# HelixDB/helix-db

Hardware: AMD Instinct MI355X
Metric: QPS @ recall@10>=0.95, 1Mx768 fp32; achieved HBM GB/s vs roofline (higher is better)
Workload: dtype f32; 1 GPU; configs[1]: 1000000x768 f32 per GPU, HNSW M=16/M0=32 ef_search=128 k=10, batch=1024 queries, squared-L2, strict-exhaustive beam (bit-exact vs reference CPU path), steps issued round-robin on 4 execution lanes; dataset=embedding, rows_per_gpu=1000000, rows_total=1000000, dim=768, batch=1024, k=10, ef_search=128, lanes=4, distinct_query_batches=25, exchange=single GPU, parallelism=1 GPU

## Files before the change

helix-db_amd/csrc/hvx_api.hip:

```cpp
#include <hip/hip_runtime.h>

#include <algorithm>
#include <atomic>
#include <cmath>
#include <cstdarg>
#include <cstdio>
#include <cstdlib>
#include <cstring>
#include <mutex>
#include <string>
#include <thread>
#include <vector>

#include "hvx_host.h"
#include "hvx_flat_mfma.h"

using namespace hvx;

namespace {
thread_local std::string g_err;
}

namespace hvx {
int fail(int code, const char *fmt, ...) {
// ... 88 lines not shown
    HIP_TRY(hipSetDevice(ix->device));
    HIP_TRY(hipStreamSynchronize(ix->stream));
    return HVX_OK;
}

extern "C" int hvx_index_set_occupancy(hvx_index *ix, uint32_t queries_per_simd) {
    if (!ix) return fail(HVX_ERR_INVARIANT, "null index");
    if (queries_per_simd != 1 && queries_per_simd != 2) return fail(HVX_ERR_K_RANGE, "occupancy must be 1 or 2 queries per SIMD");
    std::lock_guard<std::mutex> lock(ix->mu);
    ix->occupancy = queries_per_simd;
    return HVX_OK;
}

extern "C" int hvx_runtime_prepare(uint32_t hw_queues) {
    if (hw_queues == 0) hw_queues = 2;
    if (hw_queues > 2) return fail(HVX_ERR_K_RANGE, "hardware queue count %u outside 1..2", hw_queues);
    char buf[16];
    snprintf(buf, sizeof(buf), "%u", hw_queues);
    if (setenv("GPU_MAX_HW_QUEUES", buf, 0) != 0) return fail(HVX_ERR_INVARIANT, "setenv(GPU_MAX_HW_QUEUES) failed");
    return HVX_OK;
}

extern "C" int hvx_index_set_option(hvx_index *ix, uint32_t option, uint32_t value) {
    if (!ix) return fail(HVX_ERR_INVARIANT, "null index");
    if (option >= HVX_OPT_COUNT) return fail(HVX_ERR_INVARIANT, "unknown option %u", option);
    if (option == HVX_OPT_WAVE_LOG2CAP && value != 0 && (value < 7 || value > 15)) return fail(HVX_ERR_K_RANGE, "visited-table size must be 2^7 .. 2^15 slots");
    if (option == HVX_OPT_FLAT_FIRST_CHUNK && value != 0 && value < 1024) return fail(HVX_ERR_K_RANGE, "the first chunk holds at least 1024 rows");
    if (option == HVX_OPT_HNSW_PAIR && value > 3) return fail(HVX_ERR_K_RANGE, "pair kernel selector is 0 (one query per SIMD handles), 1 (never), 2 (always) or 3 (always, one gatherer)");
    if (option == HVX_OPT_FLAT_TILE_BUILD && value > 4) return fail(HVX_ERR_K_RANGE, "tile build is 0 (default: two 256-thread workgroups per CU; fp8 rows on the MX-scaled fp8 matrix instruction), 1, 2 or 3 (as 0) or 4 (as 0 with fp8 codes widened to bf16)");
    if (option == HVX_OPT_HNSW_SHADOW_PRUNE && value > 1) return fail(HVX_ERR_K_RANGE, "shadow pruning selector is 0 (on where a shadow exists) or 1 (off)");
    if (option == HVX_OPT_FLAT_NO_SMALLB && value > 2) return fail(HVX_ERR_K_RANGE, "small-batch selector is 0 (streaming kernels), 1 (never) or 2 (register-fragment build only)");
    if (option == HVX_OPT_FLAT_TILE_BUILD && value != 4) value = 0;
    if (option == HVX_OPT_DELETE_SEQUENTIAL && value != 1) value = 0;
    std::lock_guard<std::mutex> lock(ix->mu);
    ix->opt[option] = value;
    return HVX_OK;
}

extern "C" int hvx_index_read_rows_device(const hvx_index *cix, uint64_t row0, uint64_t n, float *d_out) {
    if (!cix || (!d_out && n)) return fail(HVX_ERR_INVARIANT, "null argument");
    hvx_index *ix = const_cast<hvx_index *>(cix);
    if (row0 > ix->dev.n || n > ix->dev.n - row0) return fail(HVX_ERR_INVARIANT, "rows [%llu, %llu) outside the index (%u rows)", (unsigned long long)row0,
                                                               (unsigned long long)(row0 + n), ix->dev.n);
    std::lock_guard<std::mutex> lock(ix->mu);
    HIP_TRY(hipSetDevice(ix->device));
    HIP_TRY(launch_read_rows(ix->dev, row0, n, d_out, ix->stream));
    HIP_TRY(hipStreamSynchronize(ix->stream));
    return HVX_OK;
}

extern "C" uint32_t hvx_index_last_scan_path(const hvx_index *ix) { return ix ? ix->last_scan_path : 0u; }

extern "C" void *hvx_index_stream(const hvx_index *ix) { return ix ? (void *)ix->stream : nullptr; }

// ... 557 lines not shown
    a.k = k;
    a.ef = ef;
    a.out_ids = d_ids;
    a.out_scores = d_scores;
    a.out_counts = d_counts;
    a.out_status = d_status;
    a.qstats = d_qstats ? d_qstats : ix->d_qstats;
    a.tie_flags = ix->d_tie;
    a.rerun_list = ix->d_tie + ix->max_batch;
    a.rerun_ctl = ix->d_tie + 2 * (size_t)ix->max_batch;
    a.prof = nullptr;
    a.wave_clock = nullptr;
    a.adaptive = ad ? 1u : 0u;
    a.ad = ad ? *ad : AdaptArgs{};
    a.build_nodes = nullptr;
    a.build_ef_upper = 0;
    a.only_flagged = 0;
    a.occupancy = ix->occupancy;
    a.pair = ix->opt[HVX_OPT_HNSW_PAIR] >= 2u || (ix->opt[HVX_OPT_HNSW_PAIR] == 0u && ix->occupancy != 2u) ? 1u : 0u;
    a.pair_gatherers = ix->opt[HVX_OPT_HNSW_PAIR] == 3u ? 1u : 0u;
    a.log2cap = ix->opt[HVX_OPT_WAVE_LOG2CAP];
    a.shadow = nullptr;
    a.shadow_err = nullptr;
    if (ad) {
        if (!hnsw_wave_adaptive_supported(a))
            return fail(HVX_ERR_UNSUPPORTED, "the non-strict search arms serve f32 rows of any dimension / metric (bf16 rows: dim in "
                        "{128,256,512,768,1024,1536}, cosine / Euclidean), neighbour rows <= 64 ids, ef <= 800");
        if (ix->bitmap_dirty) {
            HIP_TRY(hipMemsetAsync(ix->d_bitmap, 0, (size_t)ix->max_batch * ix->words_per_query * 4, ix->stream));
            ix->bitmap_dirty = false;
        }
        const bool ad_prof = tuning_env("HVX_WAVE_PROF") != nullptr && hnsw_wave_supported(a) && ix->occupancy != 2u;
        if (ad_prof) {
            if (!ix->d_prof && ix->dalloc((void **)&ix->d_prof, (size_t)ix->max_batch * 80)) return HVX_ERR_DEVICE;
            a.prof = ix->d_prof;
        }
        hipEvent_t e0 = nullptr, e1 = nullptr;
        pick_events(ix, timed, &e0, &e1, &a.wave_clock);
        if (e0) HIP_TRY(hipEventRecord(e0, ix->stream));
        HIP_TRY(launch_hnsw_wave(a, b, ix->stream));
        if (e1) HIP_TRY(hipEventRecord(e1, ix->stream));
        if (ad_prof) {
            std::vector<unsigned long long> h((size_t)b * 10);
            HIP_TRY(hipMemcpyAsync(h.data(), ix->d_prof, h.size() * 8, hipMemcpyDeviceToHost, ix->stream));
            HIP_TRY(hipStreamSynchronize(ix->stream));
            double acc[10] = {0, 0, 0, 0, 0, 0, 0, 0, 0, 0};
            for (uint32_t i = 0; i < b; ++i)
                for (int j = 0; j < 10; ++j) acc[j] += (double)h[(size_t)i * 10 + j];
            fprintf(stderr, "[hvx prof, non-strict] per query: row-wait %.0f  visited-claim %.0f  decide+select %.0f  gather+fma %.0f  predict %.0f  admit %.0f  (layer-0 loop %.0f) cycles\n",
                    acc[0] / b, acc[1] / b, acc[6] / b, acc[2] / b, acc[3] / b, acc[4] / b, acc[7] / b);
        }
        return HVX_OK;
    }
    const bool prof = tuning_env("HVX_WAVE_PROF") != nullptr;
    if (prof) {
        if (!ix->d_prof && ix->dalloc((void **)&ix->d_prof, (size_t)ix->max_batch * 80)) return HVX_ERR_DEVICE;
        a.prof = ix->d_prof;
    }
    const bool force_general = ix->opt[HVX_OPT_HNSW_GENERAL_KERNEL] != 0;
    const bool wave = !(force_general && ix->dev.dtype == HVX_F32) && hnsw_wave_supported(a);
    if (!wave && ix->dev.dtype != HVX_F32)
        return fail(HVX_ERR_UNSUPPORTED, ix->dev.dtype == HVX_FP8_E4M3 ? "fp8 rows serve the exact scan only (HNSW over fp8 rows is not built)"
                    : "bf16 rows are served by the one-wavefront-per-query kernel only (dim in {128,256,512,768,1024,1536}, rows <= 64 ids, ef <= 800)");
    if (ix->bitmap_dirty) {
        HIP_TRY(hipMemsetAsync(ix->d_bitmap, 0, (size_t)ix->max_batch * ix->words_per_query * 4, ix->stream));
        ix->bitmap_dirty = false;
    }
    if (wave && (ix->occupancy == 2 || prof) && ix->dev.dtype == HVX_F32 && ix->dev.metric == kL2 && !ix->opt[HVX_OPT_HNSW_SHADOW_PRUNE]) {
        uint16_t *sh = nullptr;
        float *se = nullptr;
        int rc = shadow_catch_up(ix, &sh, &se);
        if (rc) return rc;
        a.shadow = sh;
        a.shadow_err = se;
    }
    hipEvent_t e0 = nullptr, e1 = nullptr;
    pick_events(ix, timed, &e0, &e1, &a.wave_clock);
    if (e0) HIP_TRY(hipEventRecord(e0, ix->stream));
    if (wave) {
        HIP_TRY(launch_hnsw_wave(a, b, ix->stream));
        if (prof) {
            std::vector<unsigned long long> h((size_t)b * 10);
            HIP_TRY(hipMemcpyAsync(h.data(), ix->d_prof, h.size() * 8, hipMemcpyDeviceToHost, ix->stream));
            HIP_TRY(hipStreamSynchronize(ix->stream));
            double acc[10] = {0, 0, 0, 0, 0, 0, 0, 0, 0, 0};
            for (uint32_t i = 0; i < b; ++i)
                for (int j = 0; j < 10; ++j) acc[j] += (double)h[(size_t)i * 10 + j];
            fprintf(stderr, "[hvx prof] per query: row-wait %.0f  visited+shadow %.0f  gather+fma %.0f  predict %.0f  admit %.0f  (layer-0 loop %.0f) cycles;"
                            " fresh-candidate predictions %.1f  row-prefetch hits %.1f;  full-beam rows: shadow-pruned %.1f  scored in f32 %.1f"
                            " (pruned share %.4f)\n",
                    acc[0] / b, acc[1] / b, acc[2] / b, acc[3] / b, acc[4] / b, acc[7] / b, acc[5] / b, acc[6] / b, acc[8] / b, acc[9] / b,
                    acc[8] + acc[9] > 0 ? acc[8] / (acc[8] + acc[9]) : 0.0);
        }
    } else {
        HIP_TRY(launch_hnsw_search(a, b, ix->stream));
        ix->bitmap_dirty = true;
    }
    if (e1) HIP_TRY(hipEventRecord(e1, ix->stream));
    return HVX_OK;
}

extern "C" int hvx_index_timing_begin(hvx_index *ix, uint32_t capacity) {
    if (!ix) return fail(HVX_ERR_INVARIANT, "null index");
    std::lock_guard<std::mutex> lock(ix->mu);
    HIP_TRY(hipSetDevice(ix->device));
    while (ix->ring.size() < (size_t)capacity * 2) {
        hipEvent_t e;
        HIP_TRY(hipEventCreate(&e));
        ix->ring.push_back(e);
    }
    if (capacity > ix->wclk_cap) {
        int rc = ix->regrow((void **)&ix->d_wclk, (size_t)capacity * ix->max_batch * 2 * sizeof(unsigned long long));
        if (rc) return rc;
        ix->wclk_cap = capacity;
    }
// ... 322 lines not shown
```

helix-db_amd/csrc/hvx_hnsw_wave.h:

```cpp
#pragma once
#include <type_traits>

#include "hvx_beam.h"
#include "hvx_device.h"
#include "hvx_kernels.h"
#include "hvx_shadow_bound.h"

namespace hvx {

constexpr uint32_t kTabEmpty = 0xFFFFFFFFu;
constexpr uint32_t kTentativeBit = 0x80000000u;
constexpr uint32_t kHashedBit = 0x40000000u;

__device__ __forceinline__ uint32_t umin_dpp_row(uint32_t v) {
    uint32_t t;
    t = (uint32_t)__builtin_amdgcn_mov_dpp((int)v, 0xB1, 0xF, 0xF, true); v = v < t ? v : t;
    t = (uint32_t)__builtin_amdgcn_mov_dpp((int)v, 0x4E, 0xF, 0xF, true); v = v < t ? v : t;
    t = (uint32_t)__builtin_amdgcn_mov_dpp((int)v, 0x141, 0xF, 0xF, true); v = v < t ? v : t;
    t = (uint32_t)__builtin_amdgcn_mov_dpp((int)v, 0x140, 0xF, 0xF, true); v = v < t ? v : t;
    return v;
}
__device__ __forceinline__ uint32_t wave_umin(uint32_t v) {
    v = umin_dpp_row(v);
    uint32_t a = __builtin_amdgcn_readlane(v, 0), b = __builtin_amdgcn_readlane(v, 16);
// ... 375 lines not shown
        else if (!topk_ready) d.threshold = 1u;
        else d.threshold = (uint32_t)__builtin_popcountll(__ballot(delta <= brk_lane));
    }
    return d;
}

__device__ __forceinline__ float candidate_probability_fn(uint32_t kind, float base, uint32_t sim_bits, bool has_thr, uint32_t thr) {
    if (kind != 2u) return base;
    if (base <= 0.0f || base >= 1.0f) return base;
    const float sr = (float)(sim_bits < 64u ? sim_bits : 64u) / 64.0f;
    const float tr = has_thr ? (float)thr / 64.0f : 0.0f;
    const float t = __builtin_fmaxf(sr - tr, 0.0f);
    const float u = (1.0f - base) * t;
    return rs_clampf(base + u, base, 1.0f);
}

template <uint32_t METRIC, int R, int NK, bool BF, bool PROF, bool AD, bool ST, int OCC, bool BUILD>
__device__ __forceinline__ void hnsw_wave_query(const HnswArgs &a, const uint32_t vcap, const uint32_t q) {
    constexpr bool GEN = NK == 0;
    constexpr int NL = GEN ? 1 : (BF ? NK / 2 : NK);
    constexpr int P = NL <= 8 ? 2 : 1;
    constexpr bool kCosBfBig = BF && METRIC == kCosine && NL >= 24;
    constexpr bool kWide4 = OCC == 1 && 4 * P * NL <= 96 && !kCosBfBig;
    constexpr bool kWide2 = OCC == 1 || (2 * P * NL <= 48 && !kCosBfBig && !(AD && ((METRIC == kCosine && 2 * P * NL > 32) || (BF && 2 * P * NL >= 32))));
    extern __shared__ __attribute__((aligned(16))) char smem[];
    const DevIndex &ix = a.ix;
    const int lane = (int)threadIdx.x, grp = lane >> 3, j = lane & 7;
    const int slot = chunk_slot(j);

    Visited V;
    V.tab = reinterpret_cast<uint32_t *>(smem);
    V.cap = vcap;
    V.limit = OCC == 1 ? V.cap - (V.cap >> 2) : V.cap - (V.cap >> 3);
    V.words = a.words_per_query;
    V.bm = a.bitmap + (size_t)q * a.words_per_query;
    V.bm2 = (AD && a.bitmap2) ? a.bitmap2 + (size_t)q * a.words_per_query : nullptr;
    V.count = 0;
    V.spilled = false;
    uint32_t *fr_id = V.tab + V.cap;
    float *fr_d = reinterpret_cast<float *>(fr_id + 64);
    float *qs = fr_d + 64;
    uint32_t *rng_buf = reinterpret_cast<uint32_t *>(qs + (GEN ? ix.ld : (uint32_t)NK * 32u));

    const unsigned long long wclk0 = (a.wave_clock && !a.only_flagged) ? wall_clock64() : 0ull;
    const uint32_t status_in = BUILD ? 0u : (a.qstatus ? a.qstatus[q] : 0u);
    if (status_in != 0u || !ix.has_entry) {
        if (lane == 0) {
// ... 59 lines not shown
            else if (kWide4 && rem > 16u * P) { pass(std::integral_constant<int, kWide4 ? 3 * P : P>{}, f0, nf); f0 += 24u * P; }
            else if (kWide2 && rem > 8u * P) { pass(std::integral_constant<int, kWide2 ? 2 * P : P>{}, f0, nf); f0 += 16u * P; }
            else { pass(std::integral_constant<int, P>{}, f0, nf); f0 += 8u * P; }
        }
        __syncthreads();
    };
    auto score_one = [&](uint32_t node) __attribute__((always_inline)) -> float {
        if constexpr (GEN) {
            return __uint_as_float(__builtin_amdgcn_readlane(__float_as_uint(generic_distance(node)), 0));
        } else {
            uint32_t nd[1] = {node};
            float o[1];
            Gather<NK, 1, BF> g;
            gather_issue<NK, 1, BF, 1, METRIC == kCosine>(ix, nd, slot, g);
            gather_consume<METRIC, NK, 1, BF>(ix, qs, g, nd, slot, qhdr, qglobal, o);
            return __uint_as_float(__builtin_amdgcn_readlane(__float_as_uint(o[0]), 0));
        }
    };
    constexpr bool SP = !AD && !BUILD && !BF && !GEN && METRIC == kL2 && R <= 6 && (OCC == 2 || PROF);
    constexpr int SL = SP ? NK / 2 : 1;
    constexpr int kFL = (kWide4 ? 4 * P : (kWide2 ? 2 * P : P)) * NL;
    constexpr int kSWmax = !SP ? 1 : 8 * SL * 4 <= kFL * 3 ? 8 : 4 * SL * 4 <= kFL * 3 ? 4 : 3 * SL * 4 <= kFL * 3 ? 3 : 2 * SL * 4 <= kFL * 3 ? 2 : 1;
    const bool shadow_on = SP && a.shadow != nullptr;
    auto shadow_pass = [&](auto width, uint32_t f0, uint32_t nf) __attribute__((always_inline)) {
        constexpr int W = decltype(width)::value;
        uint32_t nd[W];
        uint4 x[W][SL];
        float e[W];
#pragma unroll
        for (int p = 0; p < W; ++p) {
            const uint32_t f = f0 + (uint32_t)(p * 8 + grp);
            nd[p] = fr_id[f < nf ? f : f0];
        }
#pragma unroll
        for (int p = 0; p < W; ++p) e[p] = a.shadow_err[nd[p]];
#pragma unroll
        for (int p = 0; p < W; ++p) {
            const uint4 *rp = reinterpret_cast<const uint4 *>(a.shadow + (size_t)nd[p] * ix.dim) + j;
#pragma unroll
            for (int k = 0; k < SL; ++k) x[p][k] = rp[k * 8];
        }
        __builtin_amdgcn_sched_barrier(0);
        float4 acc[W];
#pragma unroll
        for (int p = 0; p < W; ++p) acc[p] = make_float4(0.f, 0.f, 0.f, 0.f);
        const float4 *qp = reinterpret_cast<const float4 *>(qs) + 2 * j;
#pragma unroll
        for (int k = 0; k < SL; ++k) {
            const float4 q0 = qp[16 * k], q1 = qp[16 * k + 1];
#pragma unroll
            for (int p = 0; p < W; ++p) {
                const uint4 w = x[p][k];
                fma_chunk<kL2>(acc[p], q0, make_float4(__uint_as_float(w.x << 16), __uint_as_float(w.x & 0xFFFF0000u),
                                                       __uint_as_float(w.y << 16), __uint_as_float(w.y & 0xFFFF0000u)));
                fma_chunk<kL2>(acc[p], q1, make_float4(__uint_as_float(w.z << 16), __uint_as_float(w.z & 0xFFFF0000u),
                                                       __uint_as_float(w.w << 16), __uint_as_float(w.w & 0xFFFF0000u)));
            }
        }
#pragma unroll
        for (int p = 0; p < W; ++p) {
            float r = (acc[p].x + acc[p].y) + (acc[p].z + acc[p].w);
            r += __shfl_xor(r, 1, 8);
            r += __shfl_xor(r, 2, 8);
            r += __shfl_xor(r, 4, 8);
            const uint32_t f = f0 + (uint32_t)(p * 8 + grp);
            if (f < nf && j == 0) fr_d[f] = shadow_l2_lower_bound(r, e[p], ix.dim);
        }
    };
    auto shadow_prune = [&](uint32_t nf, float thr) __attribute__((always_inline)) -> uint32_t {
        if constexpr (SP) {
            uint32_t f0 = 0;
            while (f0 < nf) {
                const uint32_t rem = nf - f0;
                if (kSWmax >= 8 && rem > 32u) { shadow_pass(std::integral_constant<int, kSWmax >= 8 ? 8 : 1>{}, f0, nf); f0 += 64u; }
                else if (kSWmax >= 4 && rem > 24u) { shadow_pass(std::integral_constant<int, kSWmax >= 4 ? 4 : 1>{}, f0, nf); f0 += 32u; }
                else if (kSWmax >= 3 && rem > 16u) { shadow_pass(std::integral_constant<int, kSWmax >= 3 ? 3 : 1>{}, f0, nf); f0 += 24u; }
                else if (kSWmax >= 2 && rem > 8u) { shadow_pass(std::integral_constant<int, kSWmax >= 2 ? 2 : 1>{}, f0, nf); f0 += 16u; }
                else { shadow_pass(std::integral_constant<int, 1>{}, f0, nf); f0 += 8u; }
            }
            __syncthreads();
            const bool in = (uint32_t)lane < nf;
            const uint32_t id = in ? fr_id[lane] : kSentinel;
            const bool keep = in && !(fr_d[in ? lane : 0] > thr);
            const unsigned long long km = __ballot(keep);
            __syncthreads();
            if (keep) fr_id[__builtin_popcountll(km & ((1ull << lane) - 1ull))] = id;
            __syncthreads();
            return (uint32_t)__builtin_popcountll(km);
        } else {
            return nf;
        }
    };
    auto frontier_from = [&](uint32_t nid, uint32_t &deg) __attribute__((always_inline)) -> uint32_t {
        const bool valid = nid != kSentinel;
        const bool isnew = V.insert(nid, valid, lane);
        const unsigned long long um = __ballot(isnew);
        deg = (uint32_t)__builtin_popcountll(__ballot(valid));
        if (isnew) fr_id[__builtin_popcountll(um & ((1ull << lane) - 1ull))] = nid;
        __syncthreads();
        return (uint32_t)__builtin_popcountll(um);
    };

    uint32_t vslot = 0;
    bool vhashed = false;
    auto frontier_claim = [&](uint32_t nid, uint32_t &deg, unsigned long long &um) __attribute__((always_inline)) -> uint32_t {
        const bool valid = nid != kSentinel;
        const bool unseen = V.claim(nid, valid, lane, vslot, vhashed);
// ... 54 lines not shown
    }

    Beam<R> S;
    uint32_t st_exp = 0, st_nb = 0, st_vl = 0, st_dc = 0;
    bool tie_overflow = false;
    uint32_t bl = beam_top;
    auto load_row = [&](uint32_t c) __attribute__((always_inline)) -> uint32_t {
        if (!BUILD || bl == 0u) return (uint32_t)lane < ix.s0 ? ix.l0[(size_t)c * ix.s0 + (uint32_t)lane] : kSentinel;
        const uint32_t base = ix.up_base[c];
        return (uint32_t)lane < ix.su ? ix.up[(size_t)(base + bl - 1u) * ix.su + (uint32_t)lane] : kSentinel;
    };
    uint32_t dropped_unexpanded = 0;
    uint32_t ef = a.ef;
    uint32_t pf_id = kSentinel, pf_row = kSentinel;
    uint32_t pf_hash_for = kSentinel;
    unsigned long long pf_hash = 0ull;
    const bool want_hash = AD && a.ad.filtering != 0u;
    auto prefetch_hash = [&]() __attribute__((always_inline)) {
        if (AD && want_hash && pf_id != kSentinel && pf_hash_for != pf_id) {
            pf_hash = pf_row != kSentinel ? a.ad.node_hash[pf_row] : 0ull;
            pf_hash_for = pf_id;
        }
    };
    unsigned long long pt[10] = {0, 0, 0, 0, 0, 0, 0, 0, 0, 0}, t0 = 0, t1 = 0, t_begin = 0;
    auto tick = [&](int phase, bool wait) __attribute__((always_inline)) {
        if (PROF) {
            if (wait) asm volatile("s_waitcnt vmcnt(0) lgkmcnt(0)" ::: "memory");
            t1 = __builtin_readcyclecounter();
            pt[phase] += t1 - t0;
            t0 = t1;
        }
    };
    AdaptState A;
    QueryRngT<(OCC == 2 ? kRngWordsOcc2 : kRngWords)> G;
    uint64_t qh = 0;
    float brk_lane = -1.0f;
    if (AD) {
        A.fill = A.win_ex = A.win_filt = A.win_exp = A.bstate = A.bremain = A.reads = 0u;
        A.st = hvx_adaptive_stats{};
        qh = a.ad.qhash[q];
        brk_lane = a.ad.thr_break[lane];
        G.buf = rng_buf;
        const uint64_t ep = ix.ids[cur], efw = (uint64_t)a.ef;
        G.seed(qh ^ ((ep << 17) | (ep >> 47)) ^ ((efw << 7) | (efw >> 57)));
    }
  for (;;) {
    S.init();
// ... 21 lines not shown
            }
            break;
        }
        ++st_exp;
        const float dc = S.score_at(pos);
        const uint32_t c = S.id_at(pos);
        const uint32_t wlen = S.count < ef ? S.count : ef;
        float wmax = S.score_at(wlen - 1);
        if (AD && ST) { A.st.effective_beam_len_sum += wlen + A.fill; A.st.effective_beam_len_samples += 1u; }
        if (wlen + (AD ? A.fill : 0u) >= ef && dc > wmax) break;
        S.mark_expanded(pos, lane);

        uint32_t nid;
        if (c == pf_id) { nid = pf_row; if (PROF && !AD) pt[6] += 1; }
        else nid = load_row(c);
        tick(0, true);
        unsigned long long nh = 0ull;
        if (AD && want_hash) nh = c == pf_hash_for ? pf_hash : (nid != kSentinel ? a.ad.node_hash[nid] : 0ull);
        uint32_t deg;
        unsigned long long um = 0ull;
        uint32_t nf = AD ? frontier_claim(nid, deg, um) : frontier_from(nid, deg);
        st_nb += deg;
        tick(1, true);
        const uint32_t p2 = S.first_unexpanded(lane);
        uint32_t e2 = kSentinel, row2 = kSentinel;
        float s2 = inf;
        if (p2 < S.count) {
            e2 = S.id_at(p2);
            s2 = S.score_at(p2);
            row2 = load_row(e2);
        }
        pf_id = e2;
        pf_row = row2;
        if (nf == 0) { prefetch_hash(); continue; }
        if (AD) {
            const AdaptArgs &P = a.ad;
            const uint32_t nf0 = nf;
            const uint32_t node = nid;
            const unsigned long long node_h = nh;
            const bool unseen = (um >> lane) & 1ull;
            const uint32_t frank = (uint32_t)__builtin_popcountll(um & ((1ull << lane) - 1ull));
            const uint32_t kt = a.k > 1u ? a.k : 1u;
            const float delta = S.score_at((kt < wlen ? kt : wlen) - 1u);
            const AdaptDecision D = adapt_decide(P, A, ef, wlen >= kt, wlen, nf0, dc, delta, brk_lane);
            if (ST) A.st.simhash_bypass_trigger_low_yield += (D.trigger & 2u) ? 1u : 0u;
            if (ST) A.st.simhash_bypass_trigger_budget += (D.trigger & 1u) ? 1u : 0u;
            if (ST) A.st.active_sampling_ratio_sum += (double)D.base_p;
            if (ST) A.st.active_sampling_ratio_samples += 1u;
            if (ST && D.filter) { A.st.active_simhash_threshold_sum += D.threshold; A.st.active_simhash_threshold_samples += 1u; }
            bool keep = unseen;
            const bool pre_enabled = D.pre_kind != 0u;
            if (pre_enabled) {
                if (D.pre_p <= 0.0f) keep = false;
                else if (D.pre_p < 1.0f) {
                    G.ensure(lane);
                    keep = keep && G.below(G.pos + frank, D.pre_p);
                    G.pos += nf0;
// ... 50 lines not shown
                deferred = pass;
            }
            if (D.samp_p > 0.0f && !__ballot(sampled) && __ballot(deferred)) {
                const uint32_t best = 64u - wave_umin(deferred ? 64u - sim : 0xFFFFFFFFu);
                unsigned long long bm = __ballot(deferred & (sim == best));
                uint32_t idx = G.choose_index((uint32_t)__builtin_popcountll(bm), lane);
                while (idx--) bm &= bm - 1ull;
                sampled = (uint32_t)lane == (uint32_t)__builtin_ctzll(bm);
            }
            V.commit(node, sampled | vfail, vslot);
            const bool acc = sampled;
            const unsigned long long am = __ballot(acc);
            if (ST) A.st.simhash_passed_after_sampling += (uint32_t)__builtin_popcountll(__ballot(sampled));
            if (acc) fr_id[__builtin_popcountll(am & ((1ull << lane) - 1ull))] = node;
            __syncthreads();
            nf = (uint32_t)__builtin_popcountll(am);
            tick(6, true);
            if (nf == 0) { prefetch_hash(); continue; }
        }
        st_vl += nf;
        st_dc += nf;
        if (shadow_on && wlen >= ef) {
            const uint32_t nf_all = nf;
            nf = shadow_prune(nf, wmax);
            if (PROF) { pt[8] += nf_all - nf; pt[9] += nf; }
            tick(1, true);
        }
        score_frontier(nf);
        prefetch_hash();
        tick(2, true);
        const float d_l = (uint32_t)lane < nf ? fr_d[lane] : inf;
        const uint32_t id_l = (uint32_t)lane < nf ? fr_id[lane] : kSentinel;
        __syncthreads();
        {
            const uint32_t wl0 = (S.count < ef ? S.count : ef) + (AD ? A.fill : 0u);
            const bool adm = ((uint32_t)lane < nf) & ((d_l < wmax) | (wl0 < ef)) & (d_l >= 0.f) & (d_l < inf);
            const uint32_t key = adm ? __float_as_uint(d_l) : 0xFFFFFFFFu;
            const uint32_t kmin = wave_umin(key);
            if (kmin != 0xFFFFFFFFu && __uint_as_float(kmin) < s2) {
                const uint32_t pred = __builtin_amdgcn_readlane(id_l, (uint32_t)__builtin_ctzll(__ballot(key == kmin)));
                pf_id = pred;
                pf_row = load_row(pred);
                if (PROF) pt[5] += 1;
            }
        }
        tick(3, false);
        {
            float dv = d_l;
            const bool okv = (uint32_t)lane >= nf || score_valid(dv);
            if (__ballot(!okv)) { bad_score = true; break; }
            const uint32_t wl_in = (S.count < ef ? S.count : ef) + (AD ? A.fill : 0u);
            unsigned long long todo = __ballot(((uint32_t)lane < nf) & ((dv < wmax) | (wl_in < ef)));
            while (todo) {
                const uint32_t f = (uint32_t)__builtin_ctzll(todo);
                todo &= todo - 1ull;
                const float d = __uint_as_float(__builtin_amdgcn_readlane(__float_as_uint(dv), f));
                const uint32_t wl = (S.count < ef ? S.count : ef) + (AD ? A.fill : 0u);
                if (d < wmax || wl < ef) {
                    if (AD) A.fill -= (wl >= ef && A.fill > 0u) ? 1u : 0u;
                    float ds = 0.f;
                    const bool drop = S.insert(d, __builtin_amdgcn_readlane(id_l, f), lane, ds);
                    const uint32_t wl2 = S.count < ef ? S.count : ef;
                    wmax = S.score_at(wl2 - 1);
                    if (drop) {
                        ++dropped_unexpanded;
                        if (!(ds > wmax)) tie_overflow = true;
                    }
                }
            }
        }
        prefetch_hash();
        if (PROF) { t1 = __builtin_readcyclecounter(); pt[4] += t1 - t0; t0 = t1; }
    }
    if (!BUILD) break;
    {
        const uint32_t wl = bad_score ? 0u : (S.count < ef ? S.count : ef);
        const uint32_t outn = wl < a.k ? wl : a.k;
        const size_t slot0 = ((size_t)bl * gridDim.x + q) * a.k;
#pragma unroll
        for (int r = 0; r < R; ++r) {
            const uint32_t e = (uint32_t)r * 64u + (uint32_t)lane;
            if (e < outn) {
                a.out_ids[slot0 + e] = (uint64_t)(S.id[r] & ~kExpandedBit);
                a.out_scores[slot0 + e] = S.sc[r];
            }
        }
        if (lane == 0) a.out_counts[(size_t)bl * gridDim.x + q] = outn;
        if (bad_score || bl == 0u) break;
        cur = S.id_at(0) & ~kExpandedBit;
        cur_d = S.score_at(0);
        have_d = true;
        --bl;
    }
  }
    if (PROF && a.prof && lane == 0) {
        pt[7] = __builtin_readcyclecounter() - t_begin;
        for (int i = 0; i < 10; ++i) a.prof[(size_t)q * 10 + i] = pt[i];
    }

    uint32_t outn = 0;
    if (!BUILD && !bad_score) {
        const uint32_t ef = a.ef;
        const uint32_t wl = S.count < ef ? S.count : ef;
        outn = wl < a.k ? wl : a.k;
#pragma unroll
        for (int r = 0; r < R; ++r) {
            const uint32_t e = (uint32_t)r * 64u + (uint32_t)lane;
            if (e < outn) {
                a.out_ids[(size_t)q * a.k + e] = ix.ids[S.id[r] & ~kExpandedBit];
                a.out_scores[(size_t)q * a.k + e] = S.sc[r];
            }
        }
    }
    if (V.spilled) {
        for (uint32_t w = (uint32_t)lane; w < V.words; w += 64) { V.bm[w] = 0u; if (V.bm2) V.bm2[w] = 0u; }
    }
    if (lane == 0) {
        if (a.wave_clock && !a.only_flagged) { a.wave_clock[2 * (size_t)q] = wclk0; a.wave_clock[2 * (size_t)q + 1] = wall_clock64(); }
        if (!BUILD) a.out_counts[q] = outn;
        if (a.out_status) a.out_status[q] = bad_score ? 8u  : 0u;
// ... 112 lines not shown
```

helix-db_amd/csrc/hvx_kernels.h:

```cpp
#pragma once
#include <hip/hip_runtime.h>
#include <stdint.h>

#include "../../include/helix_vec.h"
#include "hvx_device.h"

namespace hvx {

struct AdaptArgs {
    const uint64_t *node_hash;
    const uint64_t *qhash;
    const float *thr_break;
    hvx_adaptive_stats *stats;
    uint32_t filtering;
    uint32_t configured;
    uint32_t sampling;
    float ratio;
    float pre_override;
    uint32_t count_reads;
    uint32_t read_budget;
    uint32_t bypass_windowed;
    uint32_t min_frontier, window_expansions;
    float min_filter_rate;
};

struct HnswArgs {
    DevIndex ix;
    const float *queries;
    const uint32_t *qstatus;
    const float *qhdr;
    uint32_t *bitmap;
    uint32_t *bitmap2;
    uint32_t words_per_query;
    uint32_t k, ef;
    uint64_t *out_ids;
    float *out_scores;
    uint32_t *out_counts;
    uint32_t *out_status;
    hvx_query_stats *qstats;
    uint32_t *tie_flags;
    uint32_t *rerun_list;
    uint32_t *rerun_ctl;
    unsigned long long *prof;
    unsigned long long *wave_clock;
    uint32_t adaptive;
    const uint32_t *build_nodes;
    uint32_t build_ef_upper;
    uint32_t only_flagged;
    uint32_t occupancy;
    uint32_t pair;
    uint32_t pair_gatherers;
    uint32_t log2cap;
    const uint16_t *shadow;
    const float *shadow_err;
    AdaptArgs ad;
};

// ... 55 lines not shown
```

helix-db_amd/pyhvx/__init__.py:

```python
from __future__ import annotations

import ctypes as C
import os
from dataclasses import dataclass

import numpy as np

_HERE = os.path.dirname(os.path.abspath(__file__))
LIB_PATH = os.environ.get("HVX_LIB_PATH") or os.path.join(os.path.dirname(_HERE), "libhelix_vec_gfx950.so")

COSINE, EUCLIDEAN, MANHATTAN = 0, 1, 2
F32, BF16, FP8_E4M3 = 0, 1, 2
KERNEL_SCALAR, KERNEL_SSE, KERNEL_AVX, KERNEL_AVX_FMA, KERNEL_NEON = 0, 1, 2, 3, 4
OK, ERR_DIMENSION, ERR_NONFINITE, ERR_ZERO_NORM, ERR_MAGNITUDE, ERR_K_RANGE, ERR_CANDIDATE_LIMIT, \
    ERR_DEVICE, ERR_INVARIANT, ERR_UNSUPPORTED, PENDING, ERR_BUSY, ERR_TIMEOUT = range(13)
DIR_OUT, DIR_IN, DIR_BOTH = 0, 1, 2

_STATUS_NAMES = {
    1: "InvalidDimension", 2: "InvalidVectorComponent", 3: "ZeroNormCosineVector",
    4: "ComponentMagnitudeExceeded", 5: "Query(result count / beam width out of range)",
    6: "Query(too many restricted candidates)", 7: "Device", 8: "InvariantViolation", 9: "Unsupported",
}


# ... 94 lines not shown
                                          "unsorted_entries", "self_loops", "out_of_range_ids", "holes", "level_violations",
                                          "degree_overflow_rows", "unreachable_l0")] + \
               [(n, C.c_uint32) for n in ("max_degree_l0", "max_degree_up", "bfs_levels_l0", "max_layer", "has_entry", "reserved")]

    def as_dict(self):
        return {n: int(getattr(self, n)) for n, _ in self._fields_ if n != "reserved"}


class AdaptiveStats(C.Structure):
    _fields_ = [(n, C.c_uint32) for n in (
        "simhash_filtered", "simhash_examined", "simhash_passed_before_sampling", "simhash_passed_after_sampling",
        "pre_simhash_sample_kept", "pre_simhash_sample_dropped", "simhash_bypass_expansions",
        "simhash_skipped_candidates", "simhash_bypass_trigger_budget", "simhash_bypass_trigger_low_yield",
        "active_simhash_threshold_sum", "active_simhash_threshold_samples", "effective_beam_len_sum",
        "effective_beam_len_samples", "active_sampling_ratio_samples", "rng_words", "txn_get_simhash_filter")] + \
        [("active_sampling_ratio_sum", C.c_double)]

    def as_dict(self):
        return {k: getattr(self, k) for k, _ in self._fields_}


OPT_HNSW_GENERAL_KERNEL, OPT_WAVE_LOG2CAP, OPT_FLAT_FORCE_VALU, OPT_FLAT_FIRST_CHUNK, OPT_FLAT_NO_TILE, OPT_FLAT_NO_FILTER, \
    OPT_FLAT_NO_FAST, OPT_FLAT_TILE_BUILD, OPT_FLAT_NO_SMALLB, OPT_HNSW_PAIR, OPT_DELETE_SEQUENTIAL, OPT_RESTRICTED_DIRECT, \
    OPT_RESTRICTED_EXACT_MIB, OPT_FLAT_NO_TAIL, OPT_HNSW_SHADOW_PRUNE = range(15)
PATH_VALU, PATH_MFMA_128, PATH_TILE_256, PATH_FILTERED, PATH_FULL_SPLIT, PATH_VALU_FALLBACK_QUERIES, PATH_WIDENED, \
    PATH_PAIR_OVERFLOW_REPEAT, PATH_SMALL_BATCH, PATH_DIRECT, PATH_EXACT_TAIL = 1, 2, 4, 8, 16, 32, 64, 128, 256, 512, 1024
RESTRICTED_AUTO, RESTRICTED_EXACT, RESTRICTED_FILTERED, RESTRICTED_REFERENCE_PLAN = 0, 1, 2, 3
TERM_NONE, TERM_EXHAUSTED, TERM_BEAM_COMPLETE, TERM_ROUTING_BUDGET, TERM_BRIDGE_BUDGET, TERM_VECTOR_BUDGET = range(6)


class RestrictedParams(C.Structure):
    _fields_ = [(n, C.c_uint32) for n in ("k", "ef", "strategy", "beam_percent", "directory_enabled", "explicit_budgets", "ef_filtered",
                                          "routing_rows", "bridge_rows", "vector_payloads", "sampled_seeds", "directory_seeds")]

    @classmethod
    def new(cls, k, ef, *, strategy=RESTRICTED_REFERENCE_PLAN, beam_percent=150, directory=True, **budgets):
        p = cls(k=k, ef=ef, strategy=strategy, beam_percent=beam_percent, directory_enabled=1 if directory else 0)
        if budgets:
            p.explicit_budgets = 1
            p.strategy = RESTRICTED_FILTERED
            for name in ("ef_filtered", "routing_rows", "bridge_rows", "vector_payloads", "sampled_seeds", "directory_seeds"):
                setattr(p, name, int(budgets.pop(name)))
            assert not budgets, budgets
        return p


    @classmethod
# ... 1222 lines not shown
```

include/helix_vec.h:

```cpp
#ifndef HELIX_VEC_H
#define HELIX_VEC_H

#include <stddef.h>
#include <stdint.h>

#ifdef __cplusplus
extern "C" {
#endif

typedef struct hvx_index hvx_index;
typedef struct hvx_csr hvx_csr;

enum hvx_metric { HVX_COSINE_HALF = 0, HVX_L2_SQUARED = 1, HVX_MANHATTAN = 2 };
enum hvx_dtype { HVX_F32 = 0, HVX_BF16 = 1, HVX_FP8_E4M3 = 2 };
enum hvx_float_kernel {
    HVX_KERNEL_SCALAR = 0,
    HVX_KERNEL_SSE = 1,
    HVX_KERNEL_AVX = 2,
    HVX_KERNEL_AVX_FMA = 3,
    HVX_KERNEL_NEON = 4
};

enum hvx_status {
    HVX_OK = 0,
// ... 51 lines not shown
                             hvx_index **out);
void hvx_index_free(hvx_index *);
int hvx_index_sync(const hvx_index *);
void *hvx_index_stream(const hvx_index *);
int hvx_index_read_rows_device(const hvx_index *, uint64_t row0, uint64_t n, float *d_out);
int hvx_index_set_stream(hvx_index *, void *hip_stream);
int hvx_index_fork(const hvx_index *, hvx_index **out);
enum hvx_option {
    HVX_OPT_HNSW_GENERAL_KERNEL = 0,
    HVX_OPT_WAVE_LOG2CAP = 1,
    HVX_OPT_FLAT_FORCE_VALU = 2,
    HVX_OPT_FLAT_FIRST_CHUNK = 3,
    HVX_OPT_FLAT_NO_TILE = 4,
    HVX_OPT_FLAT_NO_FILTER = 5,
    HVX_OPT_FLAT_NO_FAST = 6,
    HVX_OPT_FLAT_TILE_BUILD = 7,
    HVX_OPT_FLAT_NO_SMALLB = 8,
    HVX_OPT_HNSW_PAIR = 9,
    HVX_OPT_DELETE_SEQUENTIAL = 10,
    HVX_OPT_RESTRICTED_DIRECT = 11,
    HVX_OPT_RESTRICTED_EXACT_MIB = 12,
    HVX_OPT_FLAT_NO_TAIL = 13,
    HVX_OPT_HNSW_SHADOW_PRUNE = 14,
    HVX_OPT_COUNT = 15
};
int hvx_index_set_option(hvx_index *, uint32_t option, uint32_t value);
enum hvx_scan_path {
    HVX_PATH_VALU = 1, HVX_PATH_MFMA_128 = 2, HVX_PATH_TILE_256 = 4, HVX_PATH_FILTERED = 8, HVX_PATH_FULL_SPLIT = 16,
    HVX_PATH_VALU_FALLBACK_QUERIES = 32, HVX_PATH_WIDENED = 64,
    HVX_PATH_SMALL_BATCH = 256,
    HVX_PATH_PAIR_OVERFLOW_REPEAT = 128,
    HVX_PATH_DIRECT = 512,
    HVX_PATH_EXACT_TAIL = 1024
};
uint32_t hvx_index_last_scan_path(const hvx_index *);
int hvx_index_set_occupancy(hvx_index *, uint32_t queries_per_simd);
int hvx_index_timing_begin(hvx_index *, uint32_t capacity);
int hvx_index_timing_collect(hvx_index *, float *out_ms, uint32_t cap, uint32_t *out_n);
int hvx_index_wave_clocks(hvx_index *, uint64_t *out, uint32_t cap_launches, uint32_t rows_per_launch, uint32_t *out_n);

int hvx_search_batch(const hvx_index *, const float *queries , uint32_t b, uint32_t k,
                     uint32_t ef, uint64_t *out_ids , float *out_scores ,
                     uint32_t *out_counts , uint32_t *out_status ,
                     hvx_stats *stats );
int hvx_search_batch_device(const hvx_index *, const float *d_queries, uint32_t b, uint32_t k,
                            uint32_t ef, uint64_t *d_out_ids, float *d_out_scores,
                            uint32_t *d_out_counts, uint32_t *d_out_status,
// ... 293 lines not shown
```

Baseline: 1.430 million queries/s.

## Defer small survivor gathers into the next step's shadow pre-pass

When few frontier rows survive shadow pruning and their lower bounds cannot beat the next candidate, the full-precision gather for those survivors is postponed. It is issued alongside the next iteration's shadow-row loads, which removes a separate dependent memory round trip per step. The deferred scores are admitted into the beam before that step's pruning, and the next expansion is re-predicted afterwards. This adds register pressure and control complexity in the hot loop. It also narrows the wide-gather setting for one cosine configuration and adds profiling counters plus an option to turn the deferral off.

```diff
diff --git a/helix-db_amd/csrc/hvx_api.hip b/helix-db_amd/csrc/hvx_api.hip
--- a/helix-db_amd/csrc/hvx_api.hip
+++ b/helix-db_amd/csrc/hvx_api.hip
@@ -134,14 +134,15 @@
 }
 
 extern "C" int hvx_index_set_option(hvx_index *ix, uint32_t option, uint32_t value) {
-    if (!ix) return fail(HVX_ERR_INVARIANT, "null index");
     if (option >= HVX_OPT_COUNT) return fail(HVX_ERR_INVARIANT, "unknown option %u", option);
     if (option == HVX_OPT_WAVE_LOG2CAP && value != 0 && (value < 7 || value > 15)) return fail(HVX_ERR_K_RANGE, "visited-table size must be 2^7 .. 2^15 slots");
     if (option == HVX_OPT_FLAT_FIRST_CHUNK && value != 0 && value < 1024) return fail(HVX_ERR_K_RANGE, "the first chunk holds at least 1024 rows");
     if (option == HVX_OPT_HNSW_PAIR && value > 3) return fail(HVX_ERR_K_RANGE, "pair kernel selector is 0 (one query per SIMD handles), 1 (never), 2 (always) or 3 (always, one gatherer)");
     if (option == HVX_OPT_FLAT_TILE_BUILD && value > 4) return fail(HVX_ERR_K_RANGE, "tile build is 0 (default: two 256-thread workgroups per CU; fp8 rows on the MX-scaled fp8 matrix instruction), 1, 2 or 3 (as 0) or 4 (as 0 with fp8 codes widened to bf16)");
     if (option == HVX_OPT_HNSW_SHADOW_PRUNE && value > 1) return fail(HVX_ERR_K_RANGE, "shadow pruning selector is 0 (on where a shadow exists) or 1 (off)");
+    if (option == HVX_OPT_HNSW_DEFER_SURVIVORS && value > 1) return fail(HVX_ERR_K_RANGE, "deferred survivors selector is 0 (on where the shadow pre-pass is on) or 1 (off)");
     if (option == HVX_OPT_FLAT_NO_SMALLB && value > 2) return fail(HVX_ERR_K_RANGE, "small-batch selector is 0 (streaming kernels), 1 (never) or 2 (register-fragment build only)");
+    if (!ix) return fail(HVX_ERR_INVARIANT, "null index");
     if (option == HVX_OPT_FLAT_TILE_BUILD && value != 4) value = 0;
     if (option == HVX_OPT_DELETE_SEQUENTIAL && value != 1) value = 0;
     std::lock_guard<std::mutex> lock(ix->mu);
@@ -745,6 +746,7 @@
     a.log2cap = ix->opt[HVX_OPT_WAVE_LOG2CAP];
     a.shadow = nullptr;
     a.shadow_err = nullptr;
+    a.defer_survivors = ix->opt[HVX_OPT_HNSW_DEFER_SURVIVORS] ? 0u : 1u;
     if (ad) {
         if (!hnsw_wave_adaptive_supported(a))
             return fail(HVX_ERR_UNSUPPORTED, "the non-strict search arms serve f32 rows of any dimension / metric (bf16 rows: dim in "
@@ -755,7 +757,7 @@
         }
         const bool ad_prof = tuning_env("HVX_WAVE_PROF") != nullptr && hnsw_wave_supported(a) && ix->occupancy != 2u;
         if (ad_prof) {
-            if (!ix->d_prof && ix->dalloc((void **)&ix->d_prof, (size_t)ix->max_batch * 80)) return HVX_ERR_DEVICE;
+            if (!ix->d_prof && ix->dalloc((void **)&ix->d_prof, (size_t)ix->max_batch * 128)) return HVX_ERR_DEVICE;
             a.prof = ix->d_prof;
         }
         hipEvent_t e0 = nullptr, e1 = nullptr;
@@ -764,12 +766,12 @@
         HIP_TRY(launch_hnsw_wave(a, b, ix->stream));
         if (e1) HIP_TRY(hipEventRecord(e1, ix->stream));
         if (ad_prof) {
-            std::vector<unsigned long long> h((size_t)b * 10);
+            std::vector<unsigned long long> h((size_t)b * 16);
             HIP_TRY(hipMemcpyAsync(h.data(), ix->d_prof, h.size() * 8, hipMemcpyDeviceToHost, ix->stream));
             HIP_TRY(hipStreamSynchronize(ix->stream));
-            double acc[10] = {0, 0, 0, 0, 0, 0, 0, 0, 0, 0};
+            double acc[16] = {0, 0, 0, 0, 0, 0, 0, 0, 0, 0, 0, 0, 0, 0, 0, 0};
             for (uint32_t i = 0; i < b; ++i)
-                for (int j = 0; j < 10; ++j) acc[j] += (double)h[(size_t)i * 10 + j];
+                for (int j = 0; j < 16; ++j) acc[j] += (double)h[(size_t)i * 16 + j];
             fprintf(stderr, "[hvx prof, non-strict] per query: row-wait %.0f  visited-claim %.0f  decide+select %.0f  gather+fma %.0f  predict %.0f  admit %.0f  (layer-0 loop %.0f) cycles\n",
                     acc[0] / b, acc[1] / b, acc[6] / b, acc[2] / b, acc[3] / b, acc[4] / b, acc[7] / b);
         }
@@ -777,7 +779,7 @@
     }
     const bool prof = tuning_env("HVX_WAVE_PROF") != nullptr;
     if (prof) {
-        if (!ix->d_prof && ix->dalloc((void **)&ix->d_prof, (size_t)ix->max_batch * 80)) return HVX_ERR_DEVICE;
+        if (!ix->d_prof && ix->dalloc((void **)&ix->d_prof, (size_t)ix->max_batch * 128)) return HVX_ERR_DEVICE;
         a.prof = ix->d_prof;
     }
     const bool force_general = ix->opt[HVX_OPT_HNSW_GENERAL_KERNEL] != 0;
@@ -803,17 +805,19 @@
     if (wave) {
         HIP_TRY(launch_hnsw_wave(a, b, ix->stream));
         if (prof) {
-            std::vector<unsigned long long> h((size_t)b * 10);
+            std::vector<unsigned long long> h((size_t)b * 16);
             HIP_TRY(hipMemcpyAsync(h.data(), ix->d_prof, h.size() * 8, hipMemcpyDeviceToHost, ix->stream));
             HIP_TRY(hipStreamSynchronize(ix->stream));
-            double acc[10] = {0, 0, 0, 0, 0, 0, 0, 0, 0, 0};
+            double acc[16] = {0, 0, 0, 0, 0, 0, 0, 0, 0, 0, 0, 0, 0, 0, 0, 0};
             for (uint32_t i = 0; i < b; ++i)
-                for (int j = 0; j < 10; ++j) acc[j] += (double)h[(size_t)i * 10 + j];
+                for (int j = 0; j < 16; ++j) acc[j] += (double)h[(size_t)i * 16 + j];
             fprintf(stderr, "[hvx prof] per query: row-wait %.0f  visited+shadow %.0f  gather+fma %.0f  predict %.0f  admit %.0f  (layer-0 loop %.0f) cycles;"
                             " fresh-candidate predictions %.1f  row-prefetch hits %.1f;  full-beam rows: shadow-pruned %.1f  scored in f32 %.1f"
-                            " (pruned share %.4f)\n",
+                            " (pruned share %.4f);  survivor gathers: second trips %.1f  deferred %.1f (share %.4f)  rule failed %.1f"
+                            " (over a narrow pass %.1f  bound not clear %.1f  no next candidate / stop test %.1f)\n",
                     acc[0] / b, acc[1] / b, acc[2] / b, acc[3] / b, acc[4] / b, acc[7] / b, acc[5] / b, acc[6] / b, acc[8] / b, acc[9] / b,
-                    acc[8] + acc[9] > 0 ? acc[8] / (acc[8] + acc[9]) : 0.0);
+                    acc[8] + acc[9] > 0 ? acc[8] / (acc[8] + acc[9]) : 0.0, acc[10] / b, acc[11] / b,
+                    acc[11] + acc[12] > 0 ? acc[11] / (acc[11] + acc[12]) : 0.0, acc[12] / b, acc[13] / b, acc[14] / b, acc[15] / b);
         }
     } else {
         HIP_TRY(launch_hnsw_search(a, b, ix->stream));
diff --git a/helix-db_amd/csrc/hvx_hnsw_wave.h b/helix-db_amd/csrc/hvx_hnsw_wave.h
--- a/helix-db_amd/csrc/hvx_hnsw_wave.h
+++ b/helix-db_amd/csrc/hvx_hnsw_wave.h
@@ -1,4 +1,5 @@
 #pragma once
+#include <cassert>
 #include <type_traits>
 
 #include "hvx_beam.h"
@@ -421,7 +422,8 @@
     constexpr int P = NL <= 8 ? 2 : 1;
     constexpr bool kCosBfBig = BF && METRIC == kCosine && NL >= 24;
     constexpr bool kWide4 = OCC == 1 && 4 * P * NL <= 96 && !kCosBfBig;
-    constexpr bool kWide2 = OCC == 1 || (2 * P * NL <= 48 && !kCosBfBig && !(AD && ((METRIC == kCosine && 2 * P * NL > 32) || (BF && 2 * P * NL >= 32))));
+    constexpr bool kCosR6Big = !AD && !BF && !BUILD && METRIC == kCosine && R == 6 && NL == 24;
+    constexpr bool kWide2 = OCC == 1 || (2 * P * NL <= 48 && !kCosBfBig && !kCosR6Big && !(AD && ((METRIC == kCosine && 2 * P * NL > 32) || (BF && 2 * P * NL >= 32))));
     extern __shared__ __attribute__((aligned(16))) char smem[];
     const DevIndex &ix = a.ix;
     const int lane = (int)threadIdx.x, grp = lane >> 3, j = lane & 7;
@@ -527,11 +529,31 @@
     constexpr int kFL = (kWide4 ? 4 * P : (kWide2 ? 2 * P : P)) * NL;
     constexpr int kSWmax = !SP ? 1 : 8 * SL * 4 <= kFL * 3 ? 8 : 4 * SL * 4 <= kFL * 3 ? 4 : 3 * SL * 4 <= kFL * 3 ? 3 : 2 * SL * 4 <= kFL * 3 ? 2 : 1;
     const bool shadow_on = SP && a.shadow != nullptr;
-    auto shadow_pass = [&](auto width, uint32_t f0, uint32_t nf) __attribute__((always_inline)) {
+    constexpr int kCF = 1;
+    constexpr int kCBudget = 48;
+    constexpr int kCSfit = SP && kCBudget >= kCF * NL ? (kCBudget - kCF * NL) / SL : 0;
+    constexpr int kCS = kCSfit < kSWmax ? kCSfit : kSWmax;
+    constexpr bool kDefer = SP && kCS >= 1 && (R <= 3 || NL <= 16);
+    constexpr uint32_t kDeferOff = 0x100u;
+    uint32_t carry_n = (kDefer && shadow_on && a.defer_survivors != 0u) ? 0u : kDeferOff;
+    uint32_t carry_id = kSentinel;
+    float carry_d = 0.f;
+    auto shadow_pass = [&](auto width, auto fwidth, uint32_t f0, uint32_t nf) __attribute__((always_inline)) {
         constexpr int W = decltype(width)::value;
+        constexpr int WF = decltype(fwidth)::value, WFa = WF > 0 ? WF : 1;
         uint32_t nd[W];
         uint4 x[W][SL];
         float e[W];
+        uint32_t cn[WFa];
+        Gather<NK, WFa, false> g;
+        if constexpr (WF > 0) {
+#pragma unroll
+            for (int p = 0; p < WF; ++p) {
+                const uint32_t c = (uint32_t)(p * 8 + grp);
+                cn[p] = (uint32_t)__shfl((int)carry_id, (int)(c < carry_n ? c : 0u));
+            }
+            gather_issue<NK, WF, false>(ix, cn, slot, g);
+        }
 #pragma unroll
         for (int p = 0; p < W; ++p) {
             const uint32_t f = f0 + (uint32_t)(p * 8 + grp);
@@ -546,6 +568,15 @@
             for (int k = 0; k < SL; ++k) x[p][k] = rp[k * 8];
         }
         __builtin_amdgcn_sched_barrier(0);
+        if constexpr (WF > 0) {
+            float o[WFa];
+            gather_consume<kL2, NK, WF, false>(ix, qs, g, cn, slot, qhdr, qglobal, o);
+#pragma unroll
+            for (int p = 0; p < WF; ++p) {
+                const float t = __shfl(o[p], (lane & 7) * 8);
+                if ((lane >> 3) == p) carry_d = t;
+            }
+        }
         float4 acc[W];
 #pragma unroll
         for (int p = 0; p < W; ++p) acc[p] = make_float4(0.f, 0.f, 0.f, 0.f);
@@ -572,22 +603,28 @@
             if (f < nf && j == 0) fr_d[f] = shadow_l2_lower_bound(r, e[p], ix.dim);
         }
     };
-    auto shadow_prune = [&](uint32_t nf, float thr) __attribute__((always_inline)) -> uint32_t {
+    auto shadow_bounds = [&](uint32_t f0, uint32_t nf) __attribute__((always_inline)) {
         if constexpr (SP) {
-            uint32_t f0 = 0;
+            constexpr std::integral_constant<int, 0> nocarry{};
             while (f0 < nf) {
                 const uint32_t rem = nf - f0;
-                if (kSWmax >= 8 && rem > 32u) { shadow_pass(std::integral_constant<int, kSWmax >= 8 ? 8 : 1>{}, f0, nf); f0 += 64u; }
-                else if (kSWmax >= 4 && rem > 24u) { shadow_pass(std::integral_constant<int, kSWmax >= 4 ? 4 : 1>{}, f0, nf); f0 += 32u; }
-                else if (kSWmax >= 3 && rem > 16u) { shadow_pass(std::integral_constant<int, kSWmax >= 3 ? 3 : 1>{}, f0, nf); f0 += 24u; }
-                else if (kSWmax >= 2 && rem > 8u) { shadow_pass(std::integral_constant<int, kSWmax >= 2 ? 2 : 1>{}, f0, nf); f0 += 16u; }
-                else { shadow_pass(std::integral_constant<int, 1>{}, f0, nf); f0 += 8u; }
-            }
+                if (kSWmax >= 8 && rem > 32u) { shadow_pass(std::integral_constant<int, kSWmax >= 8 ? 8 : 1>{}, nocarry, f0, nf); f0 += 64u; }
+                else if (kSWmax >= 4 && rem > 24u) { shadow_pass(std::integral_constant<int, kSWmax >= 4 ? 4 : 1>{}, nocarry, f0, nf); f0 += 32u; }
+                else if (kSWmax >= 3 && rem > 16u) { shadow_pass(std::integral_constant<int, kSWmax >= 3 ? 3 : 1>{}, nocarry, f0, nf); f0 += 24u; }
+                else if (kSWmax >= 2 && rem > 8u) { shadow_pass(std::integral_constant<int, kSWmax >= 2 ? 2 : 1>{}, nocarry, f0, nf); f0 += 16u; }
+                else { shadow_pass(std::integral_constant<int, 1>{}, nocarry, f0, nf); f0 += 8u; }
+            }
+        }
+    };
+    auto shadow_compact = [&](uint32_t nf, float thr, float next, bool &clear) __attribute__((always_inline)) -> uint32_t {
+        if constexpr (SP) {
             __syncthreads();
             const bool in = (uint32_t)lane < nf;
             const uint32_t id = in ? fr_id[lane] : kSentinel;
-            const bool keep = in && !(fr_d[in ? lane : 0] > thr);
+            const float lb = fr_d[in ? lane : 0];
+            const bool keep = in && !(lb > thr);
             const unsigned long long km = __ballot(keep);
+            if (kDefer) clear = __ballot(keep && !(lb > next)) == 0ull;
             __syncthreads();
             if (keep) fr_id[__builtin_popcountll(km & ((1ull << lane) - 1ull))] = id;
             __syncthreads();
@@ -688,7 +725,7 @@
             pf_hash_for = pf_id;
         }
     };
-    unsigned long long pt[10] = {0, 0, 0, 0, 0, 0, 0, 0, 0, 0}, t0 = 0, t1 = 0, t_begin = 0;
+    unsigned long long pt[16] = {0, 0, 0, 0, 0, 0, 0, 0, 0, 0, 0, 0, 0, 0, 0, 0}, t0 = 0, t1 = 0, t_begin = 0;
     auto tick = [&](int phase, bool wait) __attribute__((always_inline)) {
         if (PROF) {
             if (wait) asm volatile("s_waitcnt vmcnt(0) lgkmcnt(0)" ::: "memory");
@@ -756,7 +793,7 @@
         uint32_t nf = AD ? frontier_claim(nid, deg, um) : frontier_from(nid, deg);
         st_nb += deg;
         tick(1, true);
-        const uint32_t p2 = S.first_unexpanded(lane);
+        uint32_t p2 = S.first_unexpanded(lane);
         uint32_t e2 = kSentinel, row2 = kSentinel;
         float s2 = inf;
         if (p2 < S.count) {
@@ -766,7 +803,14 @@
         }
         pf_id = e2;
         pf_row = row2;
-        if (nf == 0) { prefetch_hash(); continue; }
+        if (nf == 0) {
+            if constexpr (kDefer) {
+                if (!(carry_n & 0xFFu)) { prefetch_hash(); continue; }
+            } else {
+                prefetch_hash();
+                continue;
+            }
+        }
         if (AD) {
             const AdaptArgs &P = a.ad;
             const uint32_t nf0 = nf;
@@ -863,10 +907,79 @@
         st_dc += nf;
         if (shadow_on && wlen >= ef) {
             const uint32_t nf_all = nf;
-            nf = shadow_prune(nf, wmax);
+            bool clear = false;
+            if constexpr (kDefer) {
+                if (carry_n & 0xFFu) {
+                    const uint32_t cn = carry_n;
+                    shadow_pass(std::integral_constant<int, kDefer ? kCS : 1>{}, std::integral_constant<int, kCF>{}, 0u, nf);
+                    shadow_bounds(8u * (uint32_t)kCS, nf);
+                    carry_n = 0;
+                    if (PROF) pt[nf ? 11 : 10] += 1;
+                    tick(1, true);
+                    auto admit = [&](float dv, const uint32_t id_l, const uint32_t nf, float &wmax) __attribute__((always_inline)) -> bool {
+                        const bool okv = (uint32_t)lane >= nf || score_valid(dv);
+                        if (__ballot(!okv)) { bad_score = true; return false; }
+                        const uint32_t wl_in = (S.count < ef ? S.count : ef) + (AD ? A.fill : 0u);
+                        unsigned long long todo = __ballot(((uint32_t)lane < nf) & ((dv < wmax) | (wl_in < ef)));
+                        while (todo) {
+                            const uint32_t f = (uint32_t)__builtin_ctzll(todo);
+                            todo &= todo - 1ull;
+                            const float d = __uint_as_float(__builtin_amdgcn_readlane(__float_as_uint(dv), f));
+                            const uint32_t wl = (S.count < ef ? S.count : ef) + (AD ? A.fill : 0u);
+                            if (d < wmax || wl < ef) {
+                                if (AD) A.fill -= (wl >= ef && A.fill > 0u) ? 1u : 0u;
+                                float ds = 0.f;
+                                const bool drop = S.insert(d, __builtin_amdgcn_readlane(id_l, f), lane, ds);
+                                const uint32_t wl2 = S.count < ef ? S.count : ef;
+                                wmax = S.score_at(wl2 - 1);
+                                if (drop) {
+                                    ++dropped_unexpanded;
+                                    if (!(ds > wmax)) tie_overflow = true;
+                                }
+                            }
+                        }
+                        return true;
+                    };
+                    auto repredict = [&](uint32_t &p2, uint32_t &e2, float &s2) __attribute__((always_inline)) {
+                        p2 = S.first_unexpanded(lane);
+                        e2 = kSentinel;
+                        s2 = inf;
+                        if (p2 < S.count) {
+                            e2 = S.id_at(p2);
+                            s2 = S.score_at(p2);
+                        }
+                        if (e2 != pf_id) {
+                            pf_id = e2;
+                            pf_row = e2 != kSentinel ? load_row(e2) : kSentinel;
+                        }
+                    };
+                    if (!admit((uint32_t)lane < cn ? carry_d : inf, (uint32_t)lane < cn ? carry_id : kSentinel, cn, wmax)) break;
+                    repredict(p2, e2, s2);
+                    if (PROF) { t1 = __builtin_readcyclecounter(); pt[4] += t1 - t0; t0 = t1; }
+                } else {
+                    shadow_bounds(0u, nf);
+                }
+            } else {
+                shadow_bounds(0u, nf);
+            }
+            nf = shadow_compact(nf, wmax, s2, clear);
             if (PROF) { pt[8] += nf_all - nf; pt[9] += nf; }
             tick(1, true);
-        }
+            if constexpr (kDefer) {
+                if (nf > 0u && carry_n == 0u) {
+                    const bool c1 = p2 < S.count, c2 = nf <= 8u * (uint32_t)kCF, c4 = p2 + nf < ef;
+                    if (c1 && c2 && clear && c4) {
+                        carry_id = (uint32_t)lane < nf ? fr_id[lane] : kSentinel;
+                        carry_n = nf;
+                        __syncthreads();
+                        continue;
+                    }
+                    if (PROF) { pt[12] += 1; pt[13] += c2 ? 0 : 1; pt[14] += clear ? 0 : 1; pt[15] += (c1 && c4) ? 0 : 1; }
+                }
+            }
+            if (PROF && nf > 0u) pt[10] += 1;
+        }
+        if constexpr (kDefer) carry_id = kSentinel;
         score_frontier(nf);
         prefetch_hash();
         tick(2, true);
@@ -913,6 +1026,9 @@
         prefetch_hash();
         if (PROF) { t1 = __builtin_readcyclecounter(); pt[4] += t1 - t0; t0 = t1; }
     }
+#ifdef HVX_TUNING
+    if (PROF) assert(carry_n == 0u);
+#endif
     if (!BUILD) break;
     {
         const uint32_t wl = bad_score ? 0u : (S.count < ef ? S.count : ef);
@@ -936,7 +1052,7 @@
   }
     if (PROF && a.prof && lane == 0) {
         pt[7] = __builtin_readcyclecounter() - t_begin;
-        for (int i = 0; i < 10; ++i) a.prof[(size_t)q * 10 + i] = pt[i];
+        for (int i = 0; i < 16; ++i) a.prof[(size_t)q * 16 + i] = pt[i];
     }
 
     uint32_t outn = 0;
diff --git a/helix-db_amd/csrc/hvx_kernels.h b/helix-db_amd/csrc/hvx_kernels.h
--- a/helix-db_amd/csrc/hvx_kernels.h
+++ b/helix-db_amd/csrc/hvx_kernels.h
@@ -33,6 +33,7 @@
     uint32_t *bitmap2;
     uint32_t words_per_query;
     uint32_t k, ef;
+    uint32_t defer_survivors;
     uint64_t *out_ids;
     float *out_scores;
     uint32_t *out_counts;
diff --git a/helix-db_amd/pyhvx/__init__.py b/helix-db_amd/pyhvx/__init__.py
--- a/helix-db_amd/pyhvx/__init__.py
+++ b/helix-db_amd/pyhvx/__init__.py
@@ -140,7 +140,7 @@
 
 OPT_HNSW_GENERAL_KERNEL, OPT_WAVE_LOG2CAP, OPT_FLAT_FORCE_VALU, OPT_FLAT_FIRST_CHUNK, OPT_FLAT_NO_TILE, OPT_FLAT_NO_FILTER, \
     OPT_FLAT_NO_FAST, OPT_FLAT_TILE_BUILD, OPT_FLAT_NO_SMALLB, OPT_HNSW_PAIR, OPT_DELETE_SEQUENTIAL, OPT_RESTRICTED_DIRECT, \
-    OPT_RESTRICTED_EXACT_MIB, OPT_FLAT_NO_TAIL, OPT_HNSW_SHADOW_PRUNE = range(15)
+    OPT_RESTRICTED_EXACT_MIB, OPT_FLAT_NO_TAIL, OPT_HNSW_SHADOW_PRUNE, OPT_HNSW_DEFER_SURVIVORS = range(16)
 PATH_VALU, PATH_MFMA_128, PATH_TILE_256, PATH_FILTERED, PATH_FULL_SPLIT, PATH_VALU_FALLBACK_QUERIES, PATH_WIDENED, \
     PATH_PAIR_OVERFLOW_REPEAT, PATH_SMALL_BATCH, PATH_DIRECT, PATH_EXACT_TAIL = 1, 2, 4, 8, 16, 32, 64, 128, 256, 512, 1024
 RESTRICTED_AUTO, RESTRICTED_EXACT, RESTRICTED_FILTERED, RESTRICTED_REFERENCE_PLAN = 0, 1, 2, 3
diff --git a/include/helix_vec.h b/include/helix_vec.h
--- a/include/helix_vec.h
+++ b/include/helix_vec.h
@@ -97,7 +97,8 @@
     HVX_OPT_RESTRICTED_EXACT_MIB = 12,
     HVX_OPT_FLAT_NO_TAIL = 13,
     HVX_OPT_HNSW_SHADOW_PRUNE = 14,
-    HVX_OPT_COUNT = 15
+    HVX_OPT_HNSW_DEFER_SURVIVORS = 15,
+    HVX_OPT_COUNT = 16
 };
 int hvx_index_set_option(hvx_index *, uint32_t option, uint32_t value);
 enum hvx_scan_path {
```

New measurement: 1.370 million queries/s. -4.2%, worse.
